# zhengyk19/vit-rpe-rope

Hardware: AMD Instinct MI355X
Metric: train images/sec, CIFAR-10 ViT d=192 L=6 H=6 (higher is better)
Workload: dtype bf16; 1 GPU; CIFAR-10-shaped 32x32 patch4 ViT d=192 L=6 H=6, --pos_encoding rope-axial theta=100, bf16, full train step (fwd+CE+bwd+AdamW), random-init weights; per_gpu_batch=512, global_batch=512, parallelism=dp1, hip_graph=True

## Files before the change

vit-rpe-rope_amd/csrc/tail_cls.hip:

```cpp
#include "common.h"

namespace vitpe {

constexpr int TC_D = 192, TC_NT = 12, TC_KS = 6, TC_THREADS = 64 * TC_NT, TC_MAXHID = 1536;
constexpr int TC_XLD = TC_D + 8;
constexpr int TC_FLD = TC_D + 4;
constexpr int TC_HPAD = 8;

struct TailClsFwdArgs {
  const bf16* a;  const bf16* xin;
  const bf16* wp; const float* bp; const float* gamma; const float* beta;
  const bf16* w1; const float* b1; const bf16* w2; const float* b2;
  bf16* xmid; float* mean2; float* rstd2;
  bf16* xn_out;
  _Float16* gp_out;
  bf16* h_out;
  bf16* out;
  int B, HID, row_step;
  float eps2;
};

VITPE_DEV void tc_st4(bf16* p, const f32x4& v) { st4(p, v[0], v[1], v[2], v[3]); }

VITPE_DEV Frag<bf16> tc_phi_frag(const bf16* chunk_plus_4g) {
  const bf16x4 lo = *reinterpret_cast<const bf16x4*>(chunk_plus_4g), hi = *reinterpret_cast<const bf16x4*>(chunk_plus_4g + 16);
  Frag<bf16> f;
  f.v = __builtin_shufflevector(lo, hi, 0, 1, 2, 3, 4, 5, 6, 7);
  return f;
}

VITPE_DEV void tc_gelu(float x, float& h, float& g) {
  constexpr float C = 0.39894228040143267794f;
  const float ax = fabsf(x);
  const float T = __builtin_amdgcn_rcpf(fmaf(ax, 0.3275911f * 0.70710678118654752440f, 1.0f));
  float q = fmaf(T, 1.061405429f / (2.f * C), -1.453152027f / (2.f * C));
  q = fmaf(T, q, 1.421413741f / (2.f * C));
  q = fmaf(T, q, -0.284496736f / (2.f * C));
  q = fmaf(T, q, 0.254829592f / (2.f * C));
  const float E = __builtin_amdgcn_exp2f(fmaf(x * x, -0.72134752044448170368f, -1.32574806473615827f));
  const float H = (q * T) * E;
  h = fmaf(-ax, H, fmaxf(x, 0.f));
  const float r = fmaf(ax, E, -H);
  g = x >= 0.f ? 1.0f + r : -r;
}

__global__ __launch_bounds__(TC_THREADS) void tail_cls_fwd_kernel(TailClsFwdArgs a) {
  constexpr int D = TC_D, NT = TC_NT, KS = TC_KS;
  __shared__ __attribute__((aligned(16))) bf16 sX[16 * TC_XLD];
  __shared__ __attribute__((aligned(16))) bf16 sH[16 * (TC_MAXHID + TC_HPAD)];
  const int lane = threadIdx.x & 63, c = lane & 15, g = lane >> 4;
  const int wave = __builtin_amdgcn_readfirstlane(threadIdx.x >> 6);
  const int HID = a.HID, HLD = HID + TC_HPAD;
  const size_t row = (size_t)min(16 * (int)blockIdx.x + c, a.B - 1) * a.row_step;
  const int f0 = 16 * wave + 4 * g;

  f32x4 xm_own;
  {
    const bf16* ar = a.a + row * D + 8 * g;
    const bf16* wf = a.wp + (size_t)wave * KS * 512 + lane * 8;
    Frag<bf16> fa[KS], fw[KS];
#pragma unroll
    for (int ks = 0; ks < KS; ++ks) { fw[ks] = ld_frag(wf + ks * 512); fa[ks] = ld_frag(ar + 32 * ks); }
    const bf16x4 xr = *reinterpret_cast<const bf16x4*>(a.xin + row * D + f0);
    f32x4 acc = *reinterpret_cast<const f32x4*>(a.bp + f0);
#pragma unroll
    for (int ks = 0; ks < KS; ++ks) mma(fw[ks], fa[ks], acc);
#pragma unroll
    for (int r = 0; r < 4; ++r) acc[r] = to_f32(from_f32<bf16>(acc[r] + (float)xr[r]));
    xm_own = acc;
    tc_st4(a.xmid + row * D + f0, acc);
    tc_st4(sX + c * TC_XLD + f0, acc);
  }
  __syncthreads();

  Frag<bf16> bf[KS];
  {
    f32x4 xa[NT];
    float s1 = 0.f;
#pragma unroll
    for (int nt = 0; nt < NT; ++nt) {
      xa[nt] = ld4(sX + c * TC_XLD + 16 * nt + 4 * g);
#pragma unroll
      for (int r = 0; r < 4; ++r) s1 += xa[nt][r];
    }
    const float invD = 1.0f / (float)D;
    const float mean = xgroup_sum(s1) * invD;
    float s2 = 0.f;
#pragma unroll
    for (int nt = 0; nt < NT; ++nt)
#pragma unroll
      for (int r = 0; r < 4; ++r) { const float d = xa[nt][r] - mean; s2 += d * d; }
    const float rstd = 1.0f / sqrtf(xgroup_sum(s2) * invD + a.eps2);
    if (wave == 0 && g == 0) { a.mean2[row] = mean; a.rstd2[row] = rstd; }
#pragma unroll
    for (int nt = 0; nt < NT; ++nt) {
      const f32x4 gv = *reinterpret_cast<const f32x4*>(a.gamma + 16 * nt + 4 * g);
      const f32x4 bv = *reinterpret_cast<const f32x4*>(a.beta + 16 * nt + 4 * g);
#pragma unroll
      for (int r = 0; r < 4; ++r) xa[nt][r] = fmaf((xa[nt][r] - mean) * rstd, gv[r], bv[r]);
    }
#pragma unroll
    for (int ks = 0; ks < KS; ++ks) {
      bf[ks] = acc_to_frag<bf16>(xa[2 * ks], xa[2 * ks + 1]);
      if (a.xn_out != nullptr && ks == wave) {
        bf16* xr = a.xn_out + row * D + 32 * ks + 4 * g;
        *reinterpret_cast<bf16x4*>(xr) = __builtin_shufflevector(bf[ks].v, bf[ks].v, 0, 1, 2, 3);
        *reinterpret_cast<bf16x4*>(xr + 16) = __builtin_shufflevector(bf[ks].v, bf[ks].v, 4, 5, 6, 7);
      }
    }
  }

  const bool save = a.gp_out != nullptr;
  for (int nt = wave; nt < HID / 16; nt += NT) {
    const bf16* wf = a.w1 + (size_t)nt * KS * 512 + lane * 8;
    Frag<bf16> fw[KS];
#pragma unroll
    for (int ks = 0; ks < KS; ++ks) fw[ks] = ld_frag(wf + ks * 512);
    f32x4 acc = *reinterpret_cast<const f32x4*>(a.b1 + 16 * nt + 4 * g);
#pragma unroll
    for (int ks = 0; ks < KS; ++ks) mma(fw[ks], bf[ks], acc);
    f32x4 hh, gp;
#pragma unroll
    for (int r = 0; r < 4; ++r) { float hv, gv; tc_gelu(acc[r], hv, gv); hh[r] = hv; gp[r] = gv; }
    tc_st4(sH + c * HLD + 16 * nt + 4 * g, hh);
    if (save) {
      tc_st4(a.h_out + row * HID + 16 * nt + 4 * g, hh);
      const uint2 pk = {__builtin_bit_cast(uint32_t, __builtin_amdgcn_cvt_pkrtz(gp[0], gp[1])),
                        __builtin_bit_cast(uint32_t, __builtin_amdgcn_cvt_pkrtz(gp[2], gp[3]))};
      *reinterpret_cast<uint2*>(a.gp_out + row * HID + 16 * nt + 4 * g) = pk;
    }
  }
  __syncthreads();

  {
    f32x4 acc = *reinterpret_cast<const f32x4*>(a.b2 + f0);
    const bf16* wf = a.w2 + (size_t)wave * 512 + lane * 8;
    const bf16* hr = sH + c * HLD + 4 * g;
    for (int kc = 0; kc < HID / 32; ++kc) mma(ld_frag(wf + (size_t)kc * NT * 512), tc_phi_frag(hr + 32 * kc), acc);
#pragma unroll
    for (int r = 0; r < 4; ++r) acc[r] += xm_own[r];
    tc_st4(a.out + row * D + f0, acc);
  }
}

struct TailClsBwdArgs {
  const bf16* dy; const _Float16* gp; const bf16* xmid; const float* mean2; const float* rstd2; const float* gamma;
  const bf16* w2t; const bf16* w1t; const bf16* wpt;
  bf16* du; bf16* dxmid; bf16* da;
  float* dgamma; float* dbeta;
  int B, HID, row_step;
};

__global__ __launch_bounds__(TC_THREADS) void tail_cls_bwd_kernel(TailClsBwdArgs a) {
  constexpr int D = TC_D, NT = TC_NT, KS = TC_KS;
  __shared__ __attribute__((aligned(16))) float sDx[16 * TC_FLD];
  __shared__ __attribute__((aligned(16))) bf16 sDu[16 * (TC_MAXHID + TC_HPAD)];
  const int lane = threadIdx.x & 63, c = lane & 15, g = lane >> 4;
  const int wave = __builtin_amdgcn_readfirstlane(threadIdx.x >> 6);
  const int HID = a.HID, HLD = HID + TC_HPAD;
  const int lrow = 16 * (int)blockIdx.x + c;
  const size_t row = (size_t)min(lrow, a.B - 1) * a.row_step;
  const float valid = lrow < a.B ? 1.0f : 0.0f;
  const int f0 = 16 * wave + 4 * g;

  const bf16* const dyr = a.dy + row * D + 4 * g;
  Frag<bf16> bf[KS];
#pragma unroll
  for (int ks = 0; ks < KS; ++ks) bf[ks] = tc_phi_frag(dyr + 32 * ks);
  for (int nt = wave; nt < HID / 16; nt += NT) {
    const bf16* wf = a.w2t + (size_t)nt * KS * 512 + lane * 8;
    Frag<bf16> fw[KS];
#pragma unroll
    for (int ks = 0; ks < KS; ++ks) fw[ks] = ld_frag(wf + ks * 512);
    const uint2 gw = *reinterpret_cast<const uint2*>(a.gp + row * HID + 16 * nt + 4 * g);
    f32x4 acc = {0.f, 0.f, 0.f, 0.f};
#pragma unroll
    for (int ks = 0; ks < KS; ++ks) mma(fw[ks], bf[ks], acc);
    f32x4 d;
    d[0] = acc[0] * (float)__builtin_bit_cast(_Float16, (unsigned short)(gw.x & 0xffffu));
    d[1] = acc[1] * (float)__builtin_bit_cast(_Float16, (unsigned short)(gw.x >> 16));
    d[2] = acc[2] * (float)__builtin_bit_cast(_Float16, (unsigned short)(gw.y & 0xffffu));
    d[3] = acc[3] * (float)__builtin_bit_cast(_Float16, (unsigned short)(gw.y >> 16));
    tc_st4(a.du + row * HID + 16 * nt + 4 * g, d);
    tc_st4(sDu + c * HLD + 16 * nt + 4 * g, d);
  }
  __syncthreads();

  {
    f32x4 acc = {0.f, 0.f, 0.f, 0.f};
    const bf16* wf = a.w1t + (size_t)wave * 512 + lane * 8;
    const bf16* dr = sDu + c * HLD + 4 * g;
    for (int kc = 0; kc < HID / 32; ++kc) mma(ld_frag(wf + (size_t)kc * NT * 512), tc_phi_frag(dr + 32 * kc), acc);
    *reinterpret_cast<f32x4*>(sDx + c * TC_FLD + f0) = acc;
  }
  __syncthreads();

  f32x4 acc[NT];
  {
    const float mean = a.mean2[row], rstd = a.rstd2[row];
    const bf16* xr = a.xmid + row * D + 4 * g;
    const float invD = 1.0f / (float)D;
    bf16x4 xmv[NT];
    float s1 = 0.f, s2 = 0.f;
#pragma unroll
    for (int nt = 0; nt < NT; ++nt) {
      xmv[nt] = *reinterpret_cast<const bf16x4*>(xr + 16 * nt);
      acc[nt] = *reinterpret_cast<const f32x4*>(sDx + c * TC_FLD + 16 * nt + 4 * g);
      const f32x4 gam = *reinterpret_cast<const f32x4*>(a.gamma + 16 * nt + 4 * g);
      float tg[4], tb[4];
#pragma unroll
      for (int r = 0; r < 4; ++r) {
        const float xhat = ((float)xmv[nt][r] - mean) * rstd;
        const float dxn = acc[nt][r];
        tg[r] = dxn * xhat * valid;
        tb[r] = dxn * valid;
        const float gy = dxn * gam[r];
        s1 += gy;
        s2 = fmaf(gy, xhat, s2);
      }
      if (nt == wave) {
#pragma unroll
        for (int r = 0; r < 4; ++r) {
          const float sg = group16_sum(tg[r]), sb = group16_sum(tb[r]);
          if (c == 0) { atomicAdd(a.dgamma + 16 * nt + 4 * g + r, sg); atomicAdd(a.dbeta + 16 * nt + 4 * g + r, sb); }
        }
      }
    }
    const float m1 = xgroup_sum(s1) * invD, m2 = xgroup_sum(s2) * invD;
#pragma unroll
    for (int nt = 0; nt < NT; ++nt) {
      const bf16x4 rv = *reinterpret_cast<const bf16x4*>(dyr + 16 * nt);
      const f32x4 gam = *reinterpret_cast<const f32x4*>(a.gamma + 16 * nt + 4 * g);
#pragma unroll
      for (int r = 0; r < 4; ++r) {
        const float xhat = ((float)xmv[nt][r] - mean) * rstd;
        const float gy = acc[nt][r] * gam[r];
        acc[nt][r] = to_f32(from_f32<bf16>(fmaf(rstd, gy - m1 - xhat * m2, (float)rv[r])));
      }
      if (nt == wave) tc_st4(a.dxmid + row * D + 16 * nt + 4 * g, acc[nt]);
    }
  }

  {
    const bf16* wf = a.wpt + (size_t)wave * KS * 512 + lane * 8;
    Frag<bf16> fwp[KS];
#pragma unroll
    for (int ks = 0; ks < KS; ++ks) fwp[ks] = ld_frag(wf + ks * 512);
    f32x4 o = {0.f, 0.f, 0.f, 0.f};
#pragma unroll
    for (int ks = 0; ks < KS; ++ks) mma(fwp[ks], acc_to_frag<bf16>(acc[2 * ks], acc[2 * ks + 1]), o);
    tc_st4(a.da + row * D + f0, o);
  }
}

}

using namespace vitpe;

extern "C" int vitpe_block_tail2_supported(int dtype, int D, int HID);

extern "C" int vitpe_tail_cls_fwd(int dtype, const void* attn_out, const void* x_in, const void* Wp_packed, const float* bp,
                                  const float* gamma, const float* beta, void* x_mid, float* mean2, float* rstd2, void* xn_out,
                                  const void* W1_packed, const float* b1, const void* W2_packed, const float* b2, void* gp_out,
                                  void* h_out, void* out, float eps2, int B, int row_step, int D, int HID, hipStream_t stream) {
  VITPE_REQUIRE(attn_out && x_in && Wp_packed && bp && gamma && beta && x_mid && mean2 && rstd2 && W1_packed && b1 &&
                W2_packed && b2 && out && B >= 0 && row_step >= 1);
  VITPE_REQUIRE((gp_out == nullptr) == (h_out == nullptr));
  if (!vitpe_block_tail2_supported(dtype, D, HID)) return (int)hipErrorNotSupported;
  if (B == 0) return 0;
  TailClsFwdArgs a{};
  a.a = (const bf16*)attn_out; a.xin = (const bf16*)x_in; a.wp = (const bf16*)Wp_packed; a.bp = bp; a.gamma = gamma; a.beta = beta;
  a.w1 = (const bf16*)W1_packed; a.b1 = b1; a.w2 = (const bf16*)W2_packed; a.b2 = b2; a.xmid = (bf16*)x_mid; a.mean2 = mean2;
  a.rstd2 = rstd2; a.xn_out = (bf16*)xn_out; a.gp_out = (_Float16*)gp_out; a.h_out = (bf16*)h_out; a.out = (bf16*)out;
  a.B = B; a.HID = HID; a.row_step = row_step; a.eps2 = eps2;
  hipLaunchKernelGGL(tail_cls_fwd_kernel, dim3((B + 15) / 16), dim3(TC_THREADS), 0, stream, a);
  VITPE_CHECK_LAUNCH();
}

extern "C" int vitpe_tail_cls_bwd(int dtype, const void* dy, const void* gp, const void* W2t_packed, const void* W1t_packed,
                                  const void* x_mid, const float* mean2, const float* rstd2, const float* gamma, void* du,
                                  void* dx_mid, float* dgamma, float* dbeta, const void* WpT_packed, void* da, int B, int row_step,
                                  int D, int HID, hipStream_t stream) {
  VITPE_REQUIRE(dy && gp && W2t_packed && W1t_packed && x_mid && mean2 && rstd2 && gamma && du && dx_mid && dgamma && dbeta &&
                WpT_packed && da && B >= 0 && row_step >= 1);
  if (!vitpe_block_tail2_supported(dtype, D, HID)) return (int)hipErrorNotSupported;
  if (B == 0) return 0;
  TailClsBwdArgs a{};
  a.dy = (const bf16*)dy; a.gp = (const _Float16*)gp; a.xmid = (const bf16*)x_mid; a.mean2 = mean2; a.rstd2 = rstd2; a.gamma = gamma;
  a.w2t = (const bf16*)W2t_packed; a.w1t = (const bf16*)W1t_packed; a.wpt = (const bf16*)WpT_packed; a.du = (bf16*)du;
  a.dxmid = (bf16*)dx_mid; a.da = (bf16*)da; a.dgamma = dgamma; a.dbeta = dbeta; a.B = B; a.HID = HID; a.row_step = row_step;
  hipLaunchKernelGGL(tail_cls_bwd_kernel, dim3((B + 15) / 16), dim3(TC_THREADS), 0, stream, a);
  VITPE_CHECK_LAUNCH();
}
```

Measured before the change: 366,300 images/sec.

## Software-pipeline weight loads and restage gamma/beta in LDS for CLS tail kernels

Restructures the fused CLS-token tail forward and backward kernels so weight fragments for the next tile are loaded before the current tile's MMAs run. It double-buffers W1/W2 fragments with sched_barriers and prefetches the W2 and W1t batches ahead of the synchronisation point. Gamma/beta are staged in shared memory, and the h_out and du global stores are moved to the end, copied from LDS. The dgamma/dbeta atomics are reduced to per-wave lanes. The goal is to hide global-load latency in a small, latency-bound kernel, at the cost of higher register pressure and more complex control flow.

```diff
diff --git a/vit-rpe-rope_amd/csrc/tail_cls.hip b/vit-rpe-rope_amd/csrc/tail_cls.hip
--- a/vit-rpe-rope_amd/csrc/tail_cls.hip
+++ b/vit-rpe-rope_amd/csrc/tail_cls.hip
@@ -44,32 +44,94 @@
   g = x >= 0.f ? 1.0f + r : -r;
 }
 
+constexpr int TC_KB = 8;
+
+VITPE_DEV void tc_ld_tile(Frag<bf16> (&f)[TC_KS], const bf16* wf) {
+#pragma unroll
+  for (int ks = 0; ks < TC_KS; ++ks) f[ks] = ld_frag(wf + ks * 512);
+}
+
+VITPE_DEV void tc_ld_batch(Frag<bf16> (&f)[TC_KB], const bf16* wf, int k0, int nk) {
+#pragma unroll
+  for (int j = 0; j < TC_KB; ++j) f[j] = ld_frag(wf + (size_t)min(k0 + j, nk - 1) * (TC_NT * 512));
+}
+
+VITPE_DEV void tc_mma_batch(const Frag<bf16> (&f)[TC_KB], const bf16* src, int k0, f32x4& acc) {
+#pragma unroll
+  for (int j = 0; j < TC_KB; ++j) mma(f[j], tc_phi_frag(src + 32 * (k0 + j)), acc);
+}
+
+VITPE_DEV void tc_mma_tail(const Frag<bf16> (&f)[TC_KB], const bf16* src, int k0, int nk, f32x4& acc) {
+#pragma unroll
+  for (int j = 0; j < TC_KB; j += 2)
+    if (k0 + j < nk) {
+      mma(f[j], tc_phi_frag(src + 32 * (k0 + j)), acc);
+      mma(f[j + 1], tc_phi_frag(src + 32 * (k0 + j + 1)), acc);
+    }
+}
+
+VITPE_DEV void tc_kloop(Frag<bf16> (&fa)[TC_KB], const bf16* wf, const bf16* src, int nk, f32x4& acc) {
+  Frag<bf16> fb[TC_KB];
+  int k0 = 0;
+  for (; k0 + 2 * TC_KB < nk; k0 += 2 * TC_KB) {
+    tc_ld_batch(fb, wf, k0 + TC_KB, nk);
+    __builtin_amdgcn_sched_barrier(0);
+    tc_mma_batch(fa, src, k0, acc);
+    tc_ld_batch(fa, wf, k0 + 2 * TC_KB, nk);
+    __builtin_amdgcn_sched_barrier(0);
+    tc_mma_batch(fb, src, k0 + TC_KB, acc);
+  }
+  if (k0 + TC_KB < nk) {
+    tc_ld_batch(fb, wf, k0 + TC_KB, nk);
+    __builtin_amdgcn_sched_barrier(0);
+    tc_mma_batch(fa, src, k0, acc);
+    tc_mma_tail(fb, src, k0 + TC_KB, nk, acc);
+  } else {
+    tc_mma_tail(fa, src, k0, nk, acc);
+  }
+}
+
 __global__ __launch_bounds__(TC_THREADS) void tail_cls_fwd_kernel(TailClsFwdArgs a) {
   constexpr int D = TC_D, NT = TC_NT, KS = TC_KS;
   __shared__ __attribute__((aligned(16))) bf16 sX[16 * TC_XLD];
   __shared__ __attribute__((aligned(16))) bf16 sH[16 * (TC_MAXHID + TC_HPAD)];
-  const int lane = threadIdx.x & 63, c = lane & 15, g = lane >> 4;
-  const int wave = __builtin_amdgcn_readfirstlane(threadIdx.x >> 6);
-  const int HID = a.HID, HLD = HID + TC_HPAD;
+  __shared__ __attribute__((aligned(16))) float sGB[2 * TC_D];
+  const int tid = threadIdx.x, lane = tid & 63, c = lane & 15, g = lane >> 4;
+  const int wave = __builtin_amdgcn_readfirstlane(tid >> 6);
+  const int HID = a.HID, HLD = HID + TC_HPAD, ntiles = HID / 16, nk = HID / 32;
   const size_t row = (size_t)min(16 * (int)blockIdx.x + c, a.B - 1) * a.row_step;
   const int f0 = 16 * wave + 4 * g;
 
-  f32x4 xm_own;
+  Frag<bf16> fp[KS], fa[KS];
   {
     const bf16* ar = a.a + row * D + 8 * g;
     const bf16* wf = a.wp + (size_t)wave * KS * 512 + lane * 8;
-    Frag<bf16> fa[KS], fw[KS];
-#pragma unroll
-    for (int ks = 0; ks < KS; ++ks) { fw[ks] = ld_frag(wf + ks * 512); fa[ks] = ld_frag(ar + 32 * ks); }
-    const bf16x4 xr = *reinterpret_cast<const bf16x4*>(a.xin + row * D + f0);
-    f32x4 acc = *reinterpret_cast<const f32x4*>(a.bp + f0);
-#pragma unroll
-    for (int ks = 0; ks < KS; ++ks) mma(fw[ks], fa[ks], acc);
+#pragma unroll
+    for (int ks = 0; ks < KS; ++ks) { fp[ks] = ld_frag(wf + ks * 512); fa[ks] = ld_frag(ar + 32 * ks); }
+  }
+  const bf16x4 xr = *reinterpret_cast<const bf16x4*>(a.xin + row * D + f0);
+  const f32x4 bpv = *reinterpret_cast<const f32x4*>(a.bp + f0);
+  const f32x4 gbv = *reinterpret_cast<const f32x4*>(tid < D / 4 ? a.gamma + 4 * tid : a.beta + 4 * (min(tid, D / 2 - 1) - D / 4));
+  const bf16* const w1f = a.w1 + lane * 8;
+  const int lo = 4 * g;
+  Frag<bf16> wa[KS];
+  f32x4 ba;
+  {
+    const int nt0 = min(wave, ntiles - 1);
+    tc_ld_tile(wa, w1f + (size_t)nt0 * KS * 512);
+    ba = *reinterpret_cast<const f32x4*>(a.b1 + 16 * nt0 + lo);
+  }
+  __builtin_amdgcn_sched_barrier(0);
+
+  {
+    f32x4 acc = bpv;
+#pragma unroll
+    for (int ks = 0; ks < KS; ++ks) mma(fp[ks], fa[ks], acc);
 #pragma unroll
     for (int r = 0; r < 4; ++r) acc[r] = to_f32(from_f32<bf16>(acc[r] + (float)xr[r]));
-    xm_own = acc;
     tc_st4(a.xmid + row * D + f0, acc);
     tc_st4(sX + c * TC_XLD + f0, acc);
+    if (tid < D / 2) *reinterpret_cast<f32x4*>(sGB + 4 * tid) = gbv;
   }
   __syncthreads();
 
@@ -93,54 +155,68 @@
     const float rstd = 1.0f / sqrtf(xgroup_sum(s2) * invD + a.eps2);
     if (wave == 0 && g == 0) { a.mean2[row] = mean; a.rstd2[row] = rstd; }
 #pragma unroll
-    for (int nt = 0; nt < NT; ++nt) {
-      const f32x4 gv = *reinterpret_cast<const f32x4*>(a.gamma + 16 * nt + 4 * g);
-      const f32x4 bv = *reinterpret_cast<const f32x4*>(a.beta + 16 * nt + 4 * g);
-#pragma unroll
-      for (int r = 0; r < 4; ++r) xa[nt][r] = fmaf((xa[nt][r] - mean) * rstd, gv[r], bv[r]);
-    }
-#pragma unroll
     for (int ks = 0; ks < KS; ++ks) {
+#pragma unroll
+      for (int nt = 2 * ks; nt < 2 * ks + 2; ++nt) {
+        const f32x4 gv = *reinterpret_cast<const f32x4*>(sGB + 16 * nt + 4 * g);
+        const f32x4 bv = *reinterpret_cast<const f32x4*>(sGB + D + 16 * nt + 4 * g);
+#pragma unroll
+        for (int r = 0; r < 4; ++r) xa[nt][r] = fmaf((xa[nt][r] - mean) * rstd, gv[r], bv[r]);
+      }
       bf[ks] = acc_to_frag<bf16>(xa[2 * ks], xa[2 * ks + 1]);
       if (a.xn_out != nullptr && ks == wave) {
-        bf16* xr = a.xn_out + row * D + 32 * ks + 4 * g;
-        *reinterpret_cast<bf16x4*>(xr) = __builtin_shufflevector(bf[ks].v, bf[ks].v, 0, 1, 2, 3);
-        *reinterpret_cast<bf16x4*>(xr + 16) = __builtin_shufflevector(bf[ks].v, bf[ks].v, 4, 5, 6, 7);
+        bf16* xo = a.xn_out + row * D + 32 * ks + 4 * g;
+        *reinterpret_cast<bf16x4*>(xo) = __builtin_shufflevector(bf[ks].v, bf[ks].v, 0, 1, 2, 3);
+        *reinterpret_cast<bf16x4*>(xo + 16) = __builtin_shufflevector(bf[ks].v, bf[ks].v, 4, 5, 6, 7);
       }
-    }
-  }
+      __builtin_amdgcn_sched_barrier(0);
+    }
+  }
+
+  const bf16* const w2f = a.w2 + (size_t)wave * 512 + lane * 8;
+  Frag<bf16> f2[TC_KB];
+  tc_ld_batch(f2, w2f, 0, nk);
+  const f32x4 b2v = *reinterpret_cast<const f32x4*>(a.b2 + f0);
 
   const bool save = a.gp_out != nullptr;
-  for (int nt = wave; nt < HID / 16; nt += NT) {
-    const bf16* wf = a.w1 + (size_t)nt * KS * 512 + lane * 8;
-    Frag<bf16> fw[KS];
-#pragma unroll
-    for (int ks = 0; ks < KS; ++ks) fw[ks] = ld_frag(wf + ks * 512);
-    f32x4 acc = *reinterpret_cast<const f32x4*>(a.b1 + 16 * nt + 4 * g);
-#pragma unroll
-    for (int ks = 0; ks < KS; ++ks) mma(fw[ks], bf[ks], acc);
-    f32x4 hh, gp;
-#pragma unroll
-    for (int r = 0; r < 4; ++r) { float hv, gv; tc_gelu(acc[r], hv, gv); hh[r] = hv; gp[r] = gv; }
-    tc_st4(sH + c * HLD + 16 * nt + 4 * g, hh);
-    if (save) {
-      tc_st4(a.h_out + row * HID + 16 * nt + 4 * g, hh);
-      const uint2 pk = {__builtin_bit_cast(uint32_t, __builtin_amdgcn_cvt_pkrtz(gp[0], gp[1])),
-                        __builtin_bit_cast(uint32_t, __builtin_amdgcn_cvt_pkrtz(gp[2], gp[3]))};
-      *reinterpret_cast<uint2*>(a.gp_out + row * HID + 16 * nt + 4 * g) = pk;
-    }
+  const size_t hrow = row * HID + lo;
+  if (wave < ntiles) {
+    bf16* const shr = sH + c * HLD + lo;
+    uint2 pk = {0u, 0u};
+    for (int nt = wave; nt < ntiles; nt += NT) {
+      f32x4 acc = ba;
+#pragma unroll
+      for (int ks = 0; ks < KS; ++ks) mma(wa[ks], bf[ks], acc);
+      __builtin_amdgcn_sched_barrier(0);
+      if (nt + NT < ntiles) {
+        tc_ld_tile(wa, w1f + (size_t)(nt + NT) * KS * 512);
+        ba = *reinterpret_cast<const f32x4*>(a.b1 + 16 * (nt + NT) + lo);
+      }
+      if (save && nt != wave) *reinterpret_cast<uint2*>(a.gp_out + hrow + 16 * (nt - NT)) = pk;
+      __builtin_amdgcn_sched_barrier(0);
+      f32x4 hh, gp;
+#pragma unroll
+      for (int r = 0; r < 4; ++r) { float hv, gv; tc_gelu(acc[r], hv, gv); hh[r] = hv; gp[r] = gv; }
+      tc_st4(shr + 16 * nt, hh);
+      pk = {__builtin_bit_cast(uint32_t, __builtin_amdgcn_cvt_pkrtz(gp[0], gp[1])),
+            __builtin_bit_cast(uint32_t, __builtin_amdgcn_cvt_pkrtz(gp[2], gp[3]))};
+    }
+    if (save) *reinterpret_cast<uint2*>(a.gp_out + hrow + 16 * (wave + (ntiles - 1 - wave) / NT * NT)) = pk;
   }
   __syncthreads();
-
-  {
-    f32x4 acc = *reinterpret_cast<const f32x4*>(a.b2 + f0);
-    const bf16* wf = a.w2 + (size_t)wave * 512 + lane * 8;
-    const bf16* hr = sH + c * HLD + 4 * g;
-    for (int kc = 0; kc < HID / 32; ++kc) mma(ld_frag(wf + (size_t)kc * NT * 512), tc_phi_frag(hr + 32 * kc), acc);
+  __builtin_amdgcn_s_waitcnt(0x0F70);
+
+  {
+    f32x4 acc = b2v;
+    tc_kloop(f2, w2f, sH + c * HLD + 4 * g, nk, acc);
+    const f32x4 xm_own = ld4(sX + c * TC_XLD + f0);
 #pragma unroll
     for (int r = 0; r < 4; ++r) acc[r] += xm_own[r];
     tc_st4(a.out + row * D + f0, acc);
   }
+  if (save)
+    for (int nt = wave; nt < ntiles; nt += NT)
+      *reinterpret_cast<bf16x4*>(a.h_out + hrow + 16 * nt) = *reinterpret_cast<const bf16x4*>(sH + c * HLD + lo + 16 * nt);
 }
 
 struct TailClsBwdArgs {
@@ -151,13 +227,26 @@
   int B, HID, row_step;
 };
 
+VITPE_DEV void tc_dh_tile(const Frag<bf16> (&fw)[TC_KS], const Frag<bf16> (&bf)[TC_KS], uint2 gw, bf16* sdu) {
+  f32x4 acc = {0.f, 0.f, 0.f, 0.f};
+#pragma unroll
+  for (int ks = 0; ks < TC_KS; ++ks) mma(fw[ks], bf[ks], acc);
+  f32x4 d;
+  d[0] = acc[0] * (float)__builtin_bit_cast(_Float16, (unsigned short)(gw.x & 0xffffu));
+  d[1] = acc[1] * (float)__builtin_bit_cast(_Float16, (unsigned short)(gw.x >> 16));
+  d[2] = acc[2] * (float)__builtin_bit_cast(_Float16, (unsigned short)(gw.y & 0xffffu));
+  d[3] = acc[3] * (float)__builtin_bit_cast(_Float16, (unsigned short)(gw.y >> 16));
+  tc_st4(sdu, d);
+}
+
 __global__ __launch_bounds__(TC_THREADS) void tail_cls_bwd_kernel(TailClsBwdArgs a) {
   constexpr int D = TC_D, NT = TC_NT, KS = TC_KS;
   __shared__ __attribute__((aligned(16))) float sDx[16 * TC_FLD];
   __shared__ __attribute__((aligned(16))) bf16 sDu[16 * (TC_MAXHID + TC_HPAD)];
-  const int lane = threadIdx.x & 63, c = lane & 15, g = lane >> 4;
-  const int wave = __builtin_amdgcn_readfirstlane(threadIdx.x >> 6);
-  const int HID = a.HID, HLD = HID + TC_HPAD;
+  __shared__ __attribute__((aligned(16))) float sG[TC_D];
+  const int tid = threadIdx.x, lane = tid & 63, c = lane & 15, g = lane >> 4;
+  const int wave = __builtin_amdgcn_readfirstlane(tid >> 6);
+  const int HID = a.HID, HLD = HID + TC_HPAD, ntiles = HID / 16, nk = HID / 32;
   const int lrow = 16 * (int)blockIdx.x + c;
   const size_t row = (size_t)min(lrow, a.B - 1) * a.row_step;
   const float valid = lrow < a.B ? 1.0f : 0.0f;
@@ -167,90 +256,123 @@
   Frag<bf16> bf[KS];
 #pragma unroll
   for (int ks = 0; ks < KS; ++ks) bf[ks] = tc_phi_frag(dyr + 32 * ks);
-  for (int nt = wave; nt < HID / 16; nt += NT) {
-    const bf16* wf = a.w2t + (size_t)nt * KS * 512 + lane * 8;
-    Frag<bf16> fw[KS];
-#pragma unroll
-    for (int ks = 0; ks < KS; ++ks) fw[ks] = ld_frag(wf + ks * 512);
-    const uint2 gw = *reinterpret_cast<const uint2*>(a.gp + row * HID + 16 * nt + 4 * g);
-    f32x4 acc = {0.f, 0.f, 0.f, 0.f};
-#pragma unroll
-    for (int ks = 0; ks < KS; ++ks) mma(fw[ks], bf[ks], acc);
-    f32x4 d;
-    d[0] = acc[0] * (float)__builtin_bit_cast(_Float16, (unsigned short)(gw.x & 0xffffu));
-    d[1] = acc[1] * (float)__builtin_bit_cast(_Float16, (unsigned short)(gw.x >> 16));
-    d[2] = acc[2] * (float)__builtin_bit_cast(_Float16, (unsigned short)(gw.y & 0xffffu));
-    d[3] = acc[3] * (float)__builtin_bit_cast(_Float16, (unsigned short)(gw.y >> 16));
-    tc_st4(a.du + row * HID + 16 * nt + 4 * g, d);
-    tc_st4(sDu + c * HLD + 16 * nt + 4 * g, d);
-  }
+  const bf16* const w2f = a.w2t + lane * 8;
+  const int lo = 4 * g;
+  const size_t hrow = row * HID + lo;
+  Frag<bf16> wa[KS], wb[KS];
+  uint2 ga, gb;
+  {
+    const int nt0 = min(wave, ntiles - 1);
+    tc_ld_tile(wa, w2f + (size_t)nt0 * KS * 512);
+    ga = *reinterpret_cast<const uint2*>(a.gp + hrow + 16 * nt0);
+  }
+  const float mean = a.mean2[row], rstd = a.rstd2[row];
+  const f32x4 gmv = *reinterpret_cast<const f32x4*>(a.gamma + 4 * min(tid, D / 4 - 1));
+  const bf16x4 xown = *reinterpret_cast<const bf16x4*>(a.xmid + row * D + f0);
+  const bf16* const w1f = a.w1t + (size_t)wave * 512 + lane * 8;
+  Frag<bf16> f1[TC_KB];
+  tc_ld_batch(f1, w1f, 0, nk);
+
+  if (wave < ntiles) {
+    bf16* const sdr = sDu + c * HLD + lo;
+    int nt = wave;
+    for (; nt + 2 * NT < ntiles; nt += 2 * NT) {
+      tc_ld_tile(wb, w2f + (size_t)(nt + NT) * KS * 512);
+      gb = *reinterpret_cast<const uint2*>(a.gp + hrow + 16 * (nt + NT));
+      __builtin_amdgcn_sched_barrier(0);
+      tc_dh_tile(wa, bf, ga, sdr + 16 * nt);
+      tc_ld_tile(wa, w2f + (size_t)(nt + 2 * NT) * KS * 512);
+      ga = *reinterpret_cast<const uint2*>(a.gp + hrow + 16 * (nt + 2 * NT));
+      __builtin_amdgcn_sched_barrier(0);
+      tc_dh_tile(wb, bf, gb, sdr + 16 * (nt + NT));
+    }
+    if (nt + NT < ntiles) {
+      tc_ld_tile(wb, w2f + (size_t)(nt + NT) * KS * 512);
+      gb = *reinterpret_cast<const uint2*>(a.gp + hrow + 16 * (nt + NT));
+      __builtin_amdgcn_sched_barrier(0);
+      tc_dh_tile(wa, bf, ga, sdr + 16 * nt);
+      tc_dh_tile(wb, bf, gb, sdr + 16 * (nt + NT));
+    } else {
+      tc_dh_tile(wa, bf, ga, sdr + 16 * nt);
+    }
+  }
+  if (tid < D / 4) *reinterpret_cast<f32x4*>(sG + 4 * tid) = gmv;
   __syncthreads();
 
-  {
-    f32x4 acc = {0.f, 0.f, 0.f, 0.f};
-    const bf16* wf = a.w1t + (size_t)wave * 512 + lane * 8;
-    const bf16* dr = sDu + c * HLD + 4 * g;
-    for (int kc = 0; kc < HID / 32; ++kc) mma(ld_frag(wf + (size_t)kc * NT * 512), tc_phi_frag(dr + 32 * kc), acc);
-    *reinterpret_cast<f32x4*>(sDx + c * TC_FLD + f0) = acc;
+  bf16x4 xmv[NT];
+  {
+    const bf16* xr = a.xmid + row * D + 4 * g;
+#pragma unroll
+    for (int nt = 0; nt < NT; ++nt) xmv[nt] = *reinterpret_cast<const bf16x4*>(xr + 16 * nt);
+  }
+
+  Frag<bf16> fwp[KS];
+  bf16x4 rv[NT];
+  {
+    f32x4 dxo = {0.f, 0.f, 0.f, 0.f};
+    tc_kloop(f1, w1f, sDu + c * HLD + 4 * g, nk, dxo);
+    *reinterpret_cast<f32x4*>(sDx + c * TC_FLD + f0) = dxo;
+#pragma unroll
+    for (int nt = 0; nt < NT; ++nt) rv[nt] = *reinterpret_cast<const bf16x4*>(dyr + 16 * nt);
+    tc_ld_tile(fwp, a.wpt + (size_t)wave * KS * 512 + lane * 8);
+    float sg[4], sb[4];
+#pragma unroll
+    for (int r = 0; r < 4; ++r) {
+      const float xhat = ((float)xown[r] - mean) * rstd;
+      const float dxn = dxo[r];
+      sg[r] = group16_sum(dxn * xhat * valid);
+      sb[r] = group16_sum(dxn * valid);
+    }
+    const int qc = c & 3;
+    const float vg = qc == 0 ? sg[0] : qc == 1 ? sg[1] : qc == 2 ? sg[2] : sg[3];
+    const float vb = qc == 0 ? sb[0] : qc == 1 ? sb[1] : qc == 2 ? sb[2] : sb[3];
+    if (c < 8) atomicAdd((c < 4 ? a.dgamma : a.dbeta) + f0 + qc, c < 4 ? vg : vb);
   }
   __syncthreads();
 
   f32x4 acc[NT];
   {
-    const float mean = a.mean2[row], rstd = a.rstd2[row];
-    const bf16* xr = a.xmid + row * D + 4 * g;
     const float invD = 1.0f / (float)D;
-    bf16x4 xmv[NT];
     float s1 = 0.f, s2 = 0.f;
 #pragma unroll
+    for (int nt = 0; nt < NT; ++nt) acc[nt] = *reinterpret_cast<const f32x4*>(sDx + c * TC_FLD + 16 * nt + 4 * g);
+#pragma unroll
     for (int nt = 0; nt < NT; ++nt) {
-      xmv[nt] = *reinterpret_cast<const bf16x4*>(xr + 16 * nt);
-      acc[nt] = *reinterpret_cast<const f32x4*>(sDx + c * TC_FLD + 16 * nt + 4 * g);
-      const f32x4 gam = *reinterpret_cast<const f32x4*>(a.gamma + 16 * nt + 4 * g);
-      float tg[4], tb[4];
+      const f32x4 gam = *reinterpret_cast<const f32x4*>(sG + 16 * nt + 4 * g);
 #pragma unroll
       for (int r = 0; r < 4; ++r) {
         const float xhat = ((float)xmv[nt][r] - mean) * rstd;
-        const float dxn = acc[nt][r];
-        tg[r] = dxn * xhat * valid;
-        tb[r] = dxn * valid;
-        const float gy = dxn * gam[r];
+        const float gy = acc[nt][r] * gam[r];
         s1 += gy;
         s2 = fmaf(gy, xhat, s2);
       }
-      if (nt == wave) {
-#pragma unroll
-        for (int r = 0; r < 4; ++r) {
-          const float sg = group16_sum(tg[r]), sb = group16_sum(tb[r]);
-          if (c == 0) { atomicAdd(a.dgamma + 16 * nt + 4 * g + r, sg); atomicAdd(a.dbeta + 16 * nt + 4 * g + r, sb); }
-        }
-      }
+      if (nt % 4 == 3) __builtin_amdgcn_sched_barrier(0);
     }
     const float m1 = xgroup_sum(s1) * invD, m2 = xgroup_sum(s2) * invD;
 #pragma unroll
+    for (int nt = 0; nt < NT; ++nt) { asm volatile("" : "+v"(acc[nt])); asm volatile("" : "+v"(xmv[nt])); }
+#pragma unroll
     for (int nt = 0; nt < NT; ++nt) {
-      const bf16x4 rv = *reinterpret_cast<const bf16x4*>(dyr + 16 * nt);
-      const f32x4 gam = *reinterpret_cast<const f32x4*>(a.gamma + 16 * nt + 4 * g);
+      const f32x4 gam = *reinterpret_cast<const f32x4*>(sG + 16 * nt + 4 * g);
 #pragma unroll
       for (int r = 0; r < 4; ++r) {
         const float xhat = ((float)xmv[nt][r] - mean) * rstd;
         const float gy = acc[nt][r] * gam[r];
-        acc[nt][r] = to_f32(from_f32<bf16>(fmaf(rstd, gy - m1 - xhat * m2, (float)rv[r])));
+        acc[nt][r] = to_f32(from_f32<bf16>(fmaf(rstd, gy - m1 - xhat * m2, (float)rv[nt][r])));
       }
       if (nt == wave) tc_st4(a.dxmid + row * D + 16 * nt + 4 * g, acc[nt]);
-    }
-  }
-
-  {
-    const bf16* wf = a.wpt + (size_t)wave * KS * 512 + lane * 8;
-    Frag<bf16> fwp[KS];
-#pragma unroll
-    for (int ks = 0; ks < KS; ++ks) fwp[ks] = ld_frag(wf + ks * 512);
+      if (nt % 4 == 3) __builtin_amdgcn_sched_barrier(0);
+    }
+  }
+
+  {
     f32x4 o = {0.f, 0.f, 0.f, 0.f};
 #pragma unroll
     for (int ks = 0; ks < KS; ++ks) mma(fwp[ks], acc_to_frag<bf16>(acc[2 * ks], acc[2 * ks + 1]), o);
     tc_st4(a.da + row * D + f0, o);
   }
+  for (int nt = wave; nt < ntiles; nt += NT)
+    *reinterpret_cast<bf16x4*>(a.du + hrow + 16 * nt) = *reinterpret_cast<const bf16x4*>(sDu + c * HLD + lo + 16 * nt);
 }
 
 }
```

Measured after the change: 375,000 images/sec, median of 6. +2.4%, better.
